# bcsefercik/markerless-robot-camera-calibration

Hardware: AMD Instinct MI355X
Metric: point-cloud frames/sec at 200k pts/frame (higher is better)
Workload: dtype f32

## Files before the change

### include/sv_hip.h

```cpp
#ifndef SV_HIP_H
#define SV_HIP_H

#include <stddef.h>
#include <stdint.h>

#ifdef __cplusplus
extern "C" {
#endif

#define SV_OK 0
#define SV_ERR_INVALID (-1)
#define SV_ERR_WORKSPACE (-2)
#define SV_ERR_HIP (-3)
#define SV_ERR_RANGE (-4)
#define SV_ERR_UNSUPPORTED (-5)

#define SV_ACT_NONE 0
#define SV_ACT_RELU 1
#define SV_ACT_LEAKY_RELU 2

#define SV_POOL_MAX 0
#define SV_POOL_AVG 1

#define SV_REDUCE_MEAN 0
// ... 22 lines not shown
                  sv_stream_t stream);

size_t sv_stride_map_workspace_bytes(int64_t V_in);
int sv_stride_map(const uint64_t* keys_in, int64_t V_in, int level, void* workspace, size_t workspace_bytes,
                  uint64_t* keys_out, int32_t* vcoords_out, int32_t* parent, int32_t* child_start, int32_t* counters,
                  sv_stream_t stream);

int sv_kernel_map_k3(const int32_t* vcoords, int64_t V, int tensor_stride, int dilation, const uint64_t* table_keys,
                     const int32_t* table_vals, int64_t capacity, int32_t* nbr, int64_t ld, uint32_t* mask,
                     sv_stream_t stream);
int sv_kernel_map_down(const uint64_t* keys_fine, const int32_t* parent, int64_t V_fine, int level, int64_t V_coarse,
                       int32_t* nbr, int64_t ld, uint32_t* mask, sv_stream_t stream);
int sv_kernel_map_up(const uint64_t* keys_fine, const int32_t* parent, int64_t V_fine, int level, int32_t* nbr,
                     int64_t ld, uint32_t* mask, sv_stream_t stream);

size_t sv_plan_workspace_bytes(int64_t V);
int sv_plan_build(const int32_t* nbr, int64_t ld, const uint32_t* mask, int K, int64_t V, int64_t nbr_base, void* workspace,
                  size_t workspace_bytes, int32_t* perm, int32_t* nbr_s, uint32_t* submask, int32_t* tile_order,
                  int64_t Vpad, sv_stream_t stream);

#define SV_FRAME_MAX_LEVELS 8
#define SV_FRAME_MAX_CUTS 4
#define SV_FRAME_K3 1
#define SV_FRAME_DOWN 2
#define SV_FRAME_UP 4
#define SV_FRAME_SPLIT 8
#define SV_FRAME_RECORD 16
#define SV_FRAME_REC_HASH 1
#define SV_FRAME_REC_K3 2
#define SV_FRAME_REC_DOWN 3
#define SV_FRAME_REC_UP 4
#define SV_FRAME_REC_SPLIT 5
size_t sv_frame_maps_arena_bytes(int64_t N, int levels);
size_t sv_frame_maps_scratch_bytes(int64_t N);
int sv_frame_maps(const void* coords4, int coords_are_int, int64_t N, int levels, void* arena, size_t arena_bytes, void* scratch,
                  size_t scratch_bytes, int32_t* counters_host, int64_t* layout, sv_stream_t stream);
size_t sv_frame_plans_arena_bytes(const int64_t* V, int levels, int flags, const int32_t* split_cuts);
size_t sv_frame_plans_scratch_bytes(const int64_t* V, int levels);
int sv_frame_plans(const void* const* keys, const void* const* coords, const void* const* parent, const int64_t* V, int levels,
                   int flags, const int32_t* split_cuts, const void* const* k3_nbr, const void* const* k3_mask, void* arena,
                   size_t arena_bytes, void* scratch, size_t scratch_bytes, int64_t* layout, int max_records, sv_stream_t stream);

int sv_conv_fwd(const float* in, int64_t V_in, int64_t in_ld, int Cin, const float* W, int K, int Cout, const int32_t* perm,
                const int32_t* nbr_s, const uint32_t* submask, const int32_t* tile_order, int64_t V_out, int64_t Vpad,
                const float* scale,
                const float* shift, const float* residual, int64_t res_ld, int act, float slope, float* out,
                int64_t out_ld, sv_stream_t stream);
int sv_conv_fwd_acc(const float* in, int64_t V_in, int64_t in_ld, int Cin, const float* W, int K, int Cout, const int32_t* perm,
                    const int32_t* nbr_s, const uint32_t* submask, const int32_t* tile_order, int64_t V_out, int64_t Vpad,
                    const float* acc_init, int64_t acc_ld, const float* scale, const float* shift, const float* residual,
                    int64_t res_ld, int act, float slope, float* out, int64_t out_ld, sv_stream_t stream);
const char* sv_conv_last_instance(void);
int sv_conv_set_dispatch(double want_scale, double tail_fraction);

int sv_pack_weights_bf16(const float* W, int K, int Cin, int Cout, uint16_t* Wp, sv_stream_t stream);
int sv_conv_fwd_bf16(const float* in, int64_t V_in, int64_t in_ld, int Cin, const uint16_t* Wp, int K, int Cout,
                     const int32_t* perm, const int32_t* nbr_s, const uint32_t* submask, const int32_t* tile_order, int64_t V_out,
                     int64_t Vpad, const float* acc_init, int64_t acc_ld, const float* scale, const float* shift,
                     const float* residual, int64_t res_ld, int act, float slope, float* out, int64_t out_ld, sv_stream_t stream);

size_t sv_conv_wgrad_workspace_bytes(int64_t Vpad, int K, int Cin, int Cout);
int sv_conv_wgrad(const float* in, int64_t V_in, int64_t in_ld, int Cin, const float* dy, int64_t V_out, int64_t dy_ld,
                  int Cout, int K, const int32_t* perm, const int32_t* nbr_s, const uint32_t* submask, int64_t Vpad,
                  int accumulate, void* workspace, size_t workspace_bytes, float* dW, sv_stream_t stream);

size_t sv_conv_wgrad_bf16_workspace_bytes(int64_t Vpad, int K, int Cin, int Cout);
int sv_conv_wgrad_bf16(const float* in, int64_t V_in, int64_t in_ld, int Cin, const float* dy, int64_t V_out, int64_t dy_ld,
                       int Cout, int K, const int32_t* perm, const int32_t* nbr_s, const uint32_t* submask, int64_t Vpad,
                       int accumulate, void* workspace, size_t workspace_bytes, float* dW, sv_stream_t stream);

int sv_affine_act(const float* in, int64_t in_ld, int C, int64_t V, const float* scale, const float* shift,
                  const float* residual, int64_t res_ld, int act, float slope, float* out, int64_t out_ld,
                  sv_stream_t stream);

size_t sv_col_stats_workspace_bytes(int64_t N);
int sv_col_stats(const float* x, int64_t ld, int64_t N, int C, const float* sub, void* workspace, size_t workspace_bytes,
                 float* col_min, float* col_max, double* col_sum, float* max_row_norm, sv_stream_t stream);
int sv_center_scale(const float* x, int64_t ld, int64_t N, int C, const float* sub, const float* div, const float* add,
                    float* out, int64_t out_ld, sv_stream_t stream);

int sv_batch_offsets(const uint64_t* keys, int64_t V, int B, int32_t* batch_start, sv_stream_t stream);
int sv_global_pool(const float* F, int64_t ld, int C, const int32_t* batch_start, int B, int mode, float* out,
                   sv_stream_t stream);
int sv_slice_rows(const float* F, int64_t ld, int C, const int64_t* inverse, int64_t N, float* out,
                  sv_stream_t stream);
int sv_slice_argmax(const float* F, int64_t ld, int C, const int64_t* inverse, int64_t N, int64_t* label,
                    float* conf, sv_stream_t stream);
int sv_key_point_predictions(const float* logits, int64_t ld, int C, int64_t N, float conf_th, void* workspace,
                             size_t workspace_bytes, float* prob, int64_t* idx, int32_t* selected, sv_stream_t stream);

int sv_key_point_predictions_batched(const float* logits, int64_t ld, int C, const int64_t* seg_start_host, int G, float conf_th,
                                     void* workspace, size_t workspace_bytes, float* prob, int64_t* idx, int32_t* selected,
                                     sv_stream_t stream);
size_t sv_topk_workspace_bytes(int64_t N, int k);
int sv_topk_indices(const float* x, int64_t ld, int64_t N, int k, void* workspace, size_t workspace_bytes, int64_t* idx,
                    sv_stream_t stream);

int sv_kabsch_batched(const double* ref, const double* tgt, const int32_t* K, int Kmax, int B, double* R, double* t,
                      double* q_wxyz, sv_stream_t stream);
int sv_quat_avg_batched(const double* Q, const double* w, const int32_t* M, int Mmax, int B, double* out,
                        sv_stream_t stream);
int sv_add_metric_batched(const double* points, const int32_t* P, int Pmax, const double* gt_pose,
                          const double* pred_pose, int B, double* add_out, sv_stream_t stream);

size_t sv_icp_workspace_bytes(int64_t S);
int sv_icp_point2point(const float* src, int64_t S, const float* tgt, int64_t T, const double* init_T,
// ... 33 lines not shown
```

### markerless-robot-camera-calibration_amd/_lib.py

```python
import ctypes
import os
from ctypes import c_char_p, c_double, c_float, c_int, c_int64, c_size_t, c_void_p

import torch

_HERE = os.path.dirname(os.path.abspath(__file__))
ABI_VERSION = 4
LIB_PATH = os.environ.get("SVHIP_LIB") or os.path.join(_HERE, "libsvhip.so")

SV_ACT_NONE, SV_ACT_RELU, SV_ACT_LEAKY_RELU = 0, 1, 2
SV_POOL_MAX, SV_POOL_AVG = 0, 1
SV_REDUCE_MEAN, SV_REDUCE_FIRST = 0, 1
SV_TILE_ROWS = 128
SV_ERR_UNSUPPORTED = -5
SV_PN_MAX_LAYERS = 4
SV_PN_MAX_SCALES = 4
SV_BQ_MAX_RADII = 4
SV_COORD_BIAS = 1 << 17
SV_COORD_BITS = 18
SV_MAX_BATCH = 1024
SV_FRAME_MAX_LEVELS, SV_FRAME_MAX_CUTS, SV_FRAME_RECORD = 8, 4, 16
SV_FRAME_K3, SV_FRAME_DOWN, SV_FRAME_UP, SV_FRAME_SPLIT = 1, 2, 4, 8
SV_FRAME_REC_HASH, SV_FRAME_REC_K3, SV_FRAME_REC_DOWN, SV_FRAME_REC_UP, SV_FRAME_REC_SPLIT = 1, 2, 3, 4, 5


class SvHipError(RuntimeError):
    pass


_P = c_void_p
SIGNATURES = {
    "sv_last_error": (c_char_p, []),
    "sv_abi_version": (c_int, []),
    "sv_voxelize_workspace_bytes": (c_size_t, [c_int64]),
    "sv_voxelize": (c_int, [_P, c_int, c_int64, _P, c_size_t, _P, _P, _P, _P, _P, _P, _P]),
    "sv_voxel_reduce": (c_int, [_P, c_int, _P, _P, c_int64, c_int, _P, _P]),
    "sv_hash_build": (c_int, [_P, c_int64, _P, _P, c_int64, _P]),
    "sv_stride_map_workspace_bytes": (c_size_t, [c_int64]),
    "sv_stride_map": (c_int, [_P, c_int64, c_int, _P, c_size_t, _P, _P, _P, _P, _P, _P]),
    "sv_kernel_map_k3": (c_int, [_P, c_int64, c_int, c_int, _P, _P, c_int64, _P, c_int64, _P, _P]),
    "sv_kernel_map_down": (c_int, [_P, _P, c_int64, c_int, c_int64, _P, c_int64, _P, _P]),
    "sv_kernel_map_up": (c_int, [_P, _P, c_int64, c_int, _P, c_int64, _P, _P]),
    "sv_plan_workspace_bytes": (c_size_t, [c_int64]),
    "sv_plan_build": (c_int, [_P, c_int64, _P, c_int, c_int64, c_int64, _P, c_size_t, _P, _P, _P, _P, c_int64, _P]),
    "sv_conv_fwd": (
        c_int,
        [_P, c_int64, c_int64, c_int, _P, c_int, c_int, _P, _P, _P, _P, c_int64, c_int64, _P, _P, _P, c_int64, c_int,
         c_float, _P, c_int64, _P],
    ),
    "sv_conv_fwd_acc": (
        c_int,
        [_P, c_int64, c_int64, c_int, _P, c_int, c_int, _P, _P, _P, _P, c_int64, c_int64, _P, c_int64, _P, _P, _P, c_int64, c_int,
         c_float, _P, c_int64, _P],
    ),
    "sv_pack_weights_bf16": (c_int, [_P, c_int, c_int, c_int, _P, _P]),
    "sv_conv_fwd_bf16": (
        c_int,
        [_P, c_int64, c_int64, c_int, _P, c_int, c_int, _P, _P, _P, _P, c_int64, c_int64, _P, c_int64, _P, _P, _P, c_int64, c_int,
         c_float, _P, c_int64, _P],
    ),
    "sv_conv_wgrad_workspace_bytes": (c_size_t, [c_int64, c_int, c_int, c_int]),
    "sv_conv_wgrad": (
        c_int,
        [_P, c_int64, c_int64, c_int, _P, c_int64, c_int64, c_int, c_int, _P, _P, _P, c_int64, c_int, _P, c_size_t, _P, _P],
    ),
    "sv_conv_wgrad_bf16_workspace_bytes": (c_size_t, [c_int64, c_int, c_int, c_int]),
    "sv_conv_wgrad_bf16": (
        c_int,
        [_P, c_int64, c_int64, c_int, _P, c_int64, c_int64, c_int, c_int, _P, _P, _P, c_int64, c_int, _P, c_size_t, _P, _P],
    ),
    "sv_conv_last_instance": (c_char_p, []),
    "sv_conv_set_dispatch": (c_int, [c_double, c_double]),
    "sv_frame_maps_arena_bytes": (c_size_t, [c_int64, c_int]),
    "sv_frame_maps_scratch_bytes": (c_size_t, [c_int64]),
    "sv_frame_maps": (c_int, [_P, c_int, c_int64, c_int, _P, c_size_t, _P, c_size_t, _P, _P, _P]),
    "sv_frame_plans_arena_bytes": (c_size_t, [_P, c_int, c_int, _P]),
    "sv_frame_plans_scratch_bytes": (c_size_t, [_P, c_int]),
    "sv_frame_plans": (c_int, [_P, _P, _P, _P, c_int, c_int, _P, _P, _P, _P, c_size_t, _P, c_size_t, _P, c_int, _P]),
    "sv_affine_act": (c_int, [_P, c_int64, c_int, c_int64, _P, _P, _P, c_int64, c_int, c_float, _P, c_int64, _P]),
    "sv_col_stats_workspace_bytes": (c_size_t, [c_int64]),
    "sv_col_stats": (c_int, [_P, c_int64, c_int64, c_int, _P, _P, c_size_t, _P, _P, _P, _P, _P]),
    "sv_center_scale": (c_int, [_P, c_int64, c_int64, c_int, _P, _P, _P, _P, c_int64, _P]),
    "sv_batch_offsets": (c_int, [_P, c_int64, c_int, _P, _P]),
    "sv_global_pool": (c_int, [_P, c_int64, c_int, _P, c_int, c_int, _P, _P]),
    "sv_slice_rows": (c_int, [_P, c_int64, c_int, _P, c_int64, _P, _P]),
    "sv_slice_argmax": (c_int, [_P, c_int64, c_int, _P, c_int64, _P, _P, _P]),
    "sv_key_point_predictions": (c_int, [_P, c_int64, c_int, c_int64, c_float, _P, c_size_t, _P, _P, _P, _P]),
    "sv_key_point_predictions_batched": (c_int, [_P, c_int64, c_int, _P, c_int, c_float, _P, c_size_t, _P, _P, _P, _P]),
    "sv_topk_workspace_bytes": (c_size_t, [c_int64, c_int]),
    "sv_topk_indices": (c_int, [_P, c_int64, c_int64, c_int, _P, c_size_t, _P, _P]),
    "sv_kabsch_batched": (c_int, [_P, _P, _P, c_int, c_int, _P, _P, _P, _P]),
    "sv_quat_avg_batched": (c_int, [_P, _P, _P, c_int, c_int, _P, _P]),
    "sv_add_metric_batched": (c_int, [_P, _P, c_int, _P, _P, c_int, _P, _P]),
    "sv_icp_workspace_bytes": (c_size_t, [c_int64]),
    "sv_icp_point2point": (c_int, [_P, c_int64, _P, c_int64, _P, c_double, c_int, c_double, c_double, _P, c_size_t, _P, _P,
                                   _P]),
    "sv_fps": (c_int, [_P, c_int, c_int, c_int, _P, _P, _P]),
    "sv_three_nn_interpolate": (c_int, [_P, _P, _P, c_int, c_int, c_int, c_int, _P, _P]),
    "sv_cluster_workspace_bytes": (c_size_t, [c_int64]),
    "sv_single_linkage_roots": (c_int, [_P, c_int, c_int64, _P, c_int64, c_double, _P, c_size_t, _P, _P, _P]),
    "sv_select_equal": (c_int, [_P, c_int, c_int64, c_int64, _P, _P, _P, _P]),
    "sv_ball_query": (c_int, [_P, _P, c_int, c_int, c_int, c_double, c_int, _P, _P]),
    "sv_fps_segmented": (c_int, [_P, _P, _P, _P, c_int, c_int, _P, _P]),
    "sv_pointnet_sa": (c_int, [_P, _P, _P, _P, c_int, c_int, c_int, c_int, c_int, _P, _P, c_int, _P, _P]),
    "sv_ball_query_multi": (c_int, [_P, _P, c_int, c_int, c_int, c_int, _P, _P, _P, _P]),
    "sv_pointnet_sa_msg": (c_int, [_P, _P, _P, c_int, c_int, c_int, c_int, c_int, _P, _P, _P, _P, _P, _P, _P]),
}

_lib = None


def load():
    global _lib
    if _lib is not None:
        return _lib
    if not os.path.exists(LIB_PATH):
        raise SvHipError(
            f"{LIB_PATH} not found: build it with `python -c 'import __graft_entry__ as g; g.build()'` "
            "(or `make -C markerless-robot-camera-calibration_amd/csrc`). There is no CPU fallback."
        )
    lib = ctypes.CDLL(LIB_PATH)
    lib.sv_abi_version.restype = c_int
    if lib.sv_abi_version() != ABI_VERSION:
        raise SvHipError(f"{LIB_PATH} has C-ABI version {lib.sv_abi_version()}, this package binds version {ABI_VERSION}: "
                         "rebuild it (`python -c 'import __graft_entry__ as g; g.build()'`)")
# ... 53 lines not shown
```

### markerless-robot-camera-calibration_amd/csrc/sv_conv.hip

```cpp
#include <stdarg.h>
#include <stdio.h>
#include <stdlib.h>
#include <type_traits>
#include <algorithm>
#include <vector>

#include "sv_common.h"

namespace sv {

typedef float f32x4 __attribute__((ext_vector_type(4)));

struct ConvParams {
  const float* in;
  int64_t in_ld;
  int Cin;
  const float* W;
  int K;
  int Cout;
  const int32_t* perm;
  const int32_t* nbr_s;
  const uint32_t* submask;
  const int32_t* tile_order;
  int64_t V_out;
// ... 1405 lines not shown
  if (Cout > 128 && (Cout % 192 == 0 || Cout % 96 == 0 || Cout > 2048)) {
    if (Cout % 128 != 0) { list = wide3; n = 3; }
    else if (p.Cin % 128 == 0 && p.vec_a) { list = wide3_128_full; n = 3; }
    else { list = wide3_128; n = 4; }
  }
  else if (Cout > 64) { list = Cout % 64 == 0 ? wide2_64 : wide2; n = 4; }
  else if (Cout > 32) { list = c64; n = 3; }
  else if (Cout > 16) { list = c32; n = 3; }
  else { list = c16; n = 2; }
  static const Candidate f3[] = {{64, 2, 1, 3000, 3}, {32, 2, 1, 0, 3}};
  static const Candidate f32_32[] = {{64, 2, 1, 3000, 32}, {32, 2, 1, 0, 32}};
  static const Candidate f32_64[] = {{32, 4, 1, 1500, 32}, {16, 4, 1, 0, 32}};
  static const Candidate f64_64[] = {{32, 4, 1, 1500, 64}, {16, 4, 1, 0, 64}};
  static const bool no_fused = getenv("SV_CONV_NO_FUSED") != nullptr;
  if (p.K > 1 && !no_fused) {
    if (p.Cin == 3 && Cout > 16 && Cout <= 32) { list = f3; n = 2; }
    else if (p.Cin == 32 && p.vec_a && Cout == 32) { list = f32_32; n = 2; }
    else if (p.Cin == 32 && p.vec_a && Cout == 64) { list = f32_64; n = 2; }
    else if (p.Cin == 64 && p.vec_a && (Cout == 64 || Cout == 128)) { list = f64_64; n = 2; }
  }
  if (const char* f = getenv("SV_CONV_FORCE_RANGE")) {
    long long vmin = 0, vmax = 0;
    int cout = 0;
    Candidate c = {0, 0, 0, 0, 0};
    if (sscanf(f, "%lld:%lld:%d:%d,%d,%d", &vmin, &vmax, &cout, &c.tm, &c.wn, &c.nt) == 6 && p.Vpad >= vmin && p.Vpad <= vmax &&
        p.Cout == cout && p.K > 1)
      return launch_candidate(c, p, stream);
  }
  if (const char* f = getenv("SV_CONV_FORCE_DENSE")) {
    long long vmin = 0;
    int cout = 0;
    Candidate c = {0, 0, 0, 0, 0};
    if (sscanf(f, "%lld:%d:%d,%d,%d", &vmin, &cout, &c.tm, &c.wn, &c.nt) == 5 && p.Vpad >= vmin && p.Cout == cout && p.K == 1)
      return launch_candidate(c, p, stream);
  }
  if (const char* f = getenv("SV_CONV_FORCE")) {
    Candidate c = {0, 0, 0, 0, 0};
    if (sscanf(f, "%d,%d,%d,%d", &c.tm, &c.wn, &c.nt, &c.cpo) >= 3) return launch_candidate(c, p, stream);
  }
  static const double want_scale =
      getenv("SV_CONV_WANT_SCALE") ? atof(getenv("SV_CONV_WANT_SCALE")) : SV_CONV_WANT_SCALE_DEFAULT;
  static const double tail_fraction = getenv("SV_CONV_TAIL") ? atof(getenv("SV_CONV_TAIL")) : SV_CONV_TAIL_DEFAULT;
  const double ws = g_want_scale_override >= 0.0 ? g_want_scale_override : want_scale;
  const double tf = g_tail_override >= 0.0 ? g_tail_override : tail_fraction;
  for (int i = 0; i < n; ++i)
    if ((double)candidate_wgs(list[i], p) >= ws * (double)list[i].want) {
      const Candidate& c = list[i];
      if (c.tm == 64 && c.wn == 4 && c.nt == 3 && c.cpo == 0 && tf > 0.0 &&
          launch_conv_dual<64, 32, 4, 3>(p, stream, tf) == SV_OK)
        return SV_OK;
      return launch_candidate(c, p, stream);
    }
  return launch_candidate(list[n - 1], p, stream);
}

}

using namespace sv;

extern "C" const char* sv_conv_last_instance(void) { return sv::g_last_instance; }

extern "C" int sv_conv_set_dispatch(double want_scale, double tail_fraction) {
  SV_CHECK_ARG(tail_fraction < 1.0, "tail_fraction must be below 1");
  sv::g_want_scale_override = want_scale;
  sv::g_tail_override = tail_fraction;
  return SV_OK;
}

extern "C" int sv_conv_fwd(const float* in, int64_t V_in, int64_t in_ld, int Cin, const float* W, int K, int Cout,
                           const int32_t* perm, const int32_t* nbr_s, const uint32_t* submask,
                           const int32_t* tile_order, int64_t V_out, int64_t Vpad, const float* scale, const float* shift, const float* residual, int64_t res_ld,
                           int act, float slope, float* out, int64_t out_ld, sv_stream_t stream_) {
  return sv_conv_fwd_acc(in, V_in, in_ld, Cin, W, K, Cout, perm, nbr_s, submask, tile_order, V_out, Vpad, nullptr, 0, scale, shift,
                         residual, res_ld, act, slope, out, out_ld, stream_);
}

extern "C" int sv_conv_fwd_acc(const float* in, int64_t V_in, int64_t in_ld, int Cin, const float* W, int K, int Cout,
                               const int32_t* perm, const int32_t* nbr_s, const uint32_t* submask, const int32_t* tile_order,
                               int64_t V_out, int64_t Vpad, const float* acc_init, int64_t acc_ld, const float* scale,
                               const float* shift, const float* residual, int64_t res_ld, int act, float slope, float* out,
                               int64_t out_ld, sv_stream_t stream_) {
  hipStream_t stream = (hipStream_t)stream_;
  SV_CHECK_ARG(!acc_init || acc_ld >= Cout, "acc_init stride too small");
  SV_CHECK_ARG(Cin > 0 && Cout > 0 && K >= 1 && K <= 32, "bad channel / kernel volume");
  SV_CHECK_ARG(V_out >= 0 && Vpad >= V_out && Vpad % PLAN_TILE == 0, "Vpad must be a multiple of 128 >= V_out");
  SV_CHECK_ARG(in_ld >= Cin && out_ld >= Cout, "row strides too small");
  SV_CHECK_ARG(act >= SV_ACT_NONE && act <= SV_ACT_LEAKY_RELU, "bad activation");
  if (V_out == 0) return SV_OK;
  SV_CHECK_ARG(in && W && out, "null pointer");
  SV_CHECK_ARG(V_in >= 1, "V_in = rows of `in` (every index of the plan is below it)");
  const bool has_plan = perm || nbr_s || submask;
  SV_CHECK_ARG(!has_plan || (perm && nbr_s && submask), "perm, nbr_s and submask must be given together");
  SV_CHECK_ARG(has_plan || K == 1, "K > 1 needs a plan");
  SV_CHECK_ARG(!residual || res_ld >= Cout, "residual stride too small");
  ConvParams p;
  p.in = in; p.in_ld = in_ld; p.Cin = Cin; p.W = W; p.K = K; p.Cout = Cout;
  p.perm = perm; p.nbr_s = nbr_s; p.submask = submask; p.tile_order = tile_order; p.V_out = V_out; p.Vpad = Vpad;
  p.scale = scale; p.shift = shift; p.residual = residual; p.res_ld = res_ld;
  p.acc_init = acc_init; p.acc_ld = acc_ld;
  p.act = act; p.slope = slope; p.out = out; p.out_ld = out_ld;
  p.vec_a = (in_ld % 4 == 0) && (Cin % 4 == 0) && (((uintptr_t)in & 15) == 0);
  const uint64_t in_bytes = ((uint64_t)(V_in - 1) * (uint64_t)in_ld + (uint64_t)Cin) * 4u;
  const uint64_t w_bytes = (uint64_t)K * (uint64_t)Cin * (uint64_t)Cout * 4u;
  const uint64_t out_bytes = ((uint64_t)(V_out - 1) * (uint64_t)out_ld + (uint64_t)Cout) * 4u;
  const uint64_t res_bytes = residual ? ((uint64_t)(V_out - 1) * (uint64_t)res_ld + (uint64_t)Cout) * 4u : 0u;
  const uint64_t acc_bytes = acc_init ? ((uint64_t)(V_out - 1) * (uint64_t)acc_ld + (uint64_t)Cout) * 4u : 0u;
  p.buf_ok = in_bytes < BUF_LIMIT && w_bytes < BUF_LIMIT && out_bytes < BUF_LIMIT && res_bytes < BUF_LIMIT &&
             acc_bytes < BUF_LIMIT && (((uintptr_t)perm & 15) == 0);
  p.acc_bytes = p.buf_ok ? (uint32_t)acc_bytes : 0u;
  if (!p.buf_ok && !has_plan && K == 1 && w_bytes < BUF_LIMIT) {
    int64_t ld_max = in_ld > out_ld ? in_ld : out_ld;
    if (residual && res_ld > ld_max) ld_max = res_ld;
    const int64_t rows = (int64_t)((BUF_LIMIT - 4096u) / ((uint64_t)ld_max * 4u)) / PLAN_TILE * PLAN_TILE;
    if (rows >= PLAN_TILE && rows < V_out) {
      for (int64_t r0 = 0; r0 < V_out; r0 += rows) {
        const int64_t n = V_out - r0 < rows ? V_out - r0 : rows;
        const int rc = sv_conv_fwd_acc(in + r0 * in_ld, n, in_ld, Cin, W, K, Cout, nullptr, nullptr, nullptr, nullptr, n,
                                       (n + PLAN_TILE - 1) / PLAN_TILE * PLAN_TILE, acc_init ? acc_init + r0 * acc_ld : nullptr,
                                       acc_ld, scale, shift, residual ? residual + r0 * res_ld : nullptr, res_ld, act, slope,
                                       out + r0 * out_ld, out_ld, stream_);
        if (rc != SV_OK) return rc;
      }
      return SV_OK;
    }
  }
  p.in_bytes = p.buf_ok ? (uint32_t)in_bytes : 0u;
  p.w_bytes = p.buf_ok ? (uint32_t)w_bytes : 0u;
  p.out_bytes = p.buf_ok ? (uint32_t)out_bytes : 0u;
  p.res_bytes = p.buf_ok ? (uint32_t)res_bytes : 0u;
  p.ntiles = 0;
  p.ny = 0;
  p.trace = nullptr;
  p.main_blocks = 0;
  p.main_tiles128 = 0;
  static const bool no_first = getenv("SV_CONV_NO_FIRST") != nullptr;
  static const bool first_valu = getenv("SV_CONV_FIRST_VALU") != nullptr;
  if (has_plan && K > 1 && K <= 27 && Cin == 3 && Cout == 32 && !no_first && !acc_init) {
    if (p.buf_ok && !first_valu) return launch_conv_first_mfma(p, stream);
    return launch_conv_first_layer(p, stream);
  }
  static const bool no_thin = getenv("SV_CONV_NO_THIN") != nullptr;
  if (has_plan && K > 1 && K <= 32 && Cin == 32 && Cout == 32 && p.vec_a && p.buf_ok && !no_thin && !acc_init) return launch_conv_thin(p, stream);
  static const bool no_narrow = getenv("SV_CONV_NO_NARROW") != nullptr;
  if (!has_plan && K == 1 && Cout <= 4 && p.vec_a && Cin >= 64 && !no_narrow && !acc_init) return launch_linear_narrow(p, stream);
  return select_and_launch(p, stream);
}
```

### markerless-robot-camera-calibration_amd/model/robotnet_segmentation.py

```python
import torch.nn as nn

from .. import MinkowskiEngine as ME
from .._lib import SV_ACT_LEAKY_RELU
from ..utils import config
from ._select import pose_backbone, segmentation_backbone

EPS = 1e-6


def _classification_head(UNet, default_classes, class_name):
    class _Head(UNet):
        name = "robotnet"

        def __init__(self, in_channels, out_channels=256, D=3, num_classes=None):
            UNet.__init__(self, in_channels, out_channels, D)
            if num_classes is None:
                num_classes = default_classes()
            self.leaky_relu = ME.MinkowskiLeakyReLU()
            self.regression = nn.Sequential(
                ME.MinkowskiOps.MinkowskiLinear(256, 1024),
                ME.MinkowskiLeakyReLU(),
                ME.MinkowskiOps.MinkowskiLinear(1024, num_classes),
            )
            self.sigm = ME.MinkowskiSigmoid()

        def forward(self, x):
            if isinstance(x, tuple):
                x, _joint_angles = x
            slope = self.leaky_relu.negative_slope
            out = UNet.forward(self, x, final_act=SV_ACT_LEAKY_RELU, final_slope=slope)
            out = self.regression[0].forward_fused(out, act=SV_ACT_LEAKY_RELU,
                                                   slope=self.regression[1].negative_slope)
            return self.regression[2].forward_fused(out)

    _Head.__name__ = _Head.__qualname__ = class_name
    return _Head


def make_robotnet_segmentation(backbone=None):
    return _classification_head(segmentation_backbone(backbone), lambda: config.Config().DATA.classes,
                                "RobotNetSegmentation")


def make_robotnet_vote(backbone=None):
    return _classification_head(pose_backbone(backbone, "ROTATION"),
                                lambda: 2 if config.Config().DATA.data_type == "ee_seg" else 4, "RobotNetVote")


RobotNetSegmentation = make_robotnet_segmentation()
```

### markerless-robot-camera-calibration_amd/nn.py

```python
import math
from ctypes import c_float, c_int, c_int64, c_size_t

import numpy as np
import torch
import torch.nn as nn

from . import _lib, profiling
from ._lib import SV_ACT_LEAKY_RELU, SV_ACT_NONE, SV_ACT_RELU, call, ptr, stream_ptr
from .sparse import SparseTensor, SplitPlan

KERNEL_OFFSET_PERMUTATION = None

import os as _os


def _parse_split_rules(text):
    rules = []
    for part in text.split(";"):
        if part.strip():
            rows, _, cuts = part.partition(":")
            cuts = tuple(int(v) for v in cuts.split(",") if v)
            rules.append((int(rows), cuts[0] if len(cuts) == 1 else cuts))
    return sorted(rules, key=lambda r: -r[0])

# ... 50 lines not shown
        wp = weight_bf16[k0 * Cin * Cout:k1 * Cin * Cout] if weight_bf16 is not None else None
        if i == len(plan.parts) - 1:
            _conv_forward_one(feats, w, sub, V_out, scale, shift, residual, act, slope, out, acc, timed=False, wp=wp)
        else:
            nxt = torch.empty((V_out, Cout), dtype=torch.float32, device=feats.device)
            _conv_forward_one(feats, w, sub, V_out, None, None, None, SV_ACT_NONE, slope, nxt, acc, timed=False, wp=wp)
            acc = nxt
    if t0 is not None:
        timer.stop(t0, _lib.conv_last_instance()[0], K, Cin, Cout, V_out, plan.pairs_device(), level=plan.out_stride,
                   passes=len(plan.parts))
    return out


def _conv_forward_one(feats, weight3, plan, V_out, scale, shift, residual, act, slope, out, acc_init, timed=True, wp=None):
    K, Cin, Cout = weight3.shape
    if plan is None:
        Vpad = (max(V_out, 1) + _lib.SV_TILE_ROWS - 1) // _lib.SV_TILE_ROWS * _lib.SV_TILE_ROWS
    else:
        Vpad = plan.Vpad
    timer = profiling.TIMER if timed else None
    t0 = None
    if timer is not None:
        kname = profiling.conv_kernel_config(Cout, Vpad, Cin, K)
        if timer.want(kname):
            t0 = timer.start()
    res_ld = residual.stride(0) if residual is not None else 0

    log = profiling.INSTANCE_LOG

    acc_ld = acc_init.stride(0) if acc_init is not None else 0

    fn, w_arg = ("sv_conv_fwd_acc", weight3) if wp is None else ("sv_conv_fwd_bf16", wp)

    def launch(f, pl, o, r, v_out, v_pad, a=None):
        call(fn, ptr(f), c_int64(f.shape[0]), c_int64(f.stride(0)), c_int(Cin), ptr(w_arg), c_int(K),
             c_int(Cout), ptr(pl.perm if pl else None), ptr(pl.nbr_s if pl else None), ptr(pl.submask if pl else None),
             ptr(pl.tile_order if pl else None), c_int64(v_out), c_int64(v_pad), ptr(a), c_int64(acc_ld), ptr(scale), ptr(shift),
             ptr(r), c_int64(res_ld), c_int(act), c_float(slope), ptr(o), c_int64(o.stride(0)), stream_ptr())
        if log is not None:
            log.append((*_lib.conv_last_instance(), K, Cin, Cout, v_out))

    parts = plan.chunks(4 * feats.stride(0), 4 * max(out.stride(0), res_ld, acc_ld)) if plan is not None else None
    if parts is None:
        launch(feats, plan, out, residual, V_out, Vpad, acc_init)
    else:
        for sub, i0, i1, o0, o1 in parts:
            launch(feats[i0:i1], sub, out[o0:o1], residual[o0:o1] if residual is not None else None, o1 - o0, sub.Vpad,
                   acc_init[o0:o1] if acc_init is not None else None)
    if t0 is not None:
        timer.stop(t0, _lib.conv_last_instance()[0], K, Cin, Cout, V_out,
                   plan.pairs_device() if plan is not None else None,
                   level=plan.out_stride if plan is not None else None)
    return out


def _wgrad_one(feats, dy, plan, K, Cin, Cout, V_out, dW, accumulate, bf16=False):
    Vpad = (plan.Vpad if plan is not None
            else (max(V_out, 1) + _lib.SV_TILE_ROWS - 1) // _lib.SV_TILE_ROWS * _lib.SV_TILE_ROWS)
    lib = _lib.load()
    fn = "sv_conv_wgrad_bf16" if bf16 else "sv_conv_wgrad"
    nbytes = getattr(lib, fn + "_workspace_bytes")(c_int64(Vpad), c_int(K), c_int(Cin), c_int(Cout))
    ws = torch.empty(max(nbytes, 1), dtype=torch.uint8, device=dy.device)
    rc = getattr(lib, fn)(ptr(feats), c_int64(feats.shape[0]), c_int64(feats.stride(0)), c_int(Cin), ptr(dy),
                          c_int64(V_out), c_int64(dy.stride(0)), c_int(Cout), c_int(K), ptr(plan.perm if plan else None),
                          ptr(plan.nbr_s if plan else None), ptr(plan.submask if plan else None), c_int64(Vpad),
                          c_int(1 if accumulate else 0), ptr(ws), c_size_t(nbytes), ptr(dW), stream_ptr())
    if bf16 and rc == _lib.SV_ERR_UNSUPPORTED:
        return _wgrad_one(feats, dy, plan, K, Cin, Cout, V_out, dW, accumulate)
    _lib._check(rc, fn)
    return fn


def conv_wgrad(feats, dy, plan, K, Cin, Cout, bf16=False, used=None):
    if feats.stride(1) != 1:
        feats = feats.contiguous()
    if dy.stride(1) != 1:
        dy = dy.contiguous()
    V_out = dy.shape[0]
    dW = torch.empty((K, Cin, Cout), dtype=torch.float32, device=dy.device)
    used = set() if used is None else used
    if isinstance(plan, SplitPlan):
        for k0, k1, sub in plan.parts:
            _wgrad_plan(feats, dy, sub, k1 - k0, Cin, Cout, V_out, dW[k0:k1], bf16, used)
    else:
        _wgrad_plan(feats, dy, plan, K, Cin, Cout, V_out, dW, bf16, used)
    return dW


def _wgrad_plan(feats, dy, plan, K, Cin, Cout, V_out, dW, bf16=False, used=None):
    used = set() if used is None else used
    parts = plan.chunks(4 * feats.stride(0), 4 * dy.stride(0)) if plan is not None else None
    if parts is None:
        used.add(_wgrad_one(feats, dy, plan, K, Cin, Cout, V_out, dW, False, bf16))
        return
    for j, (sub, i0, i1, o0, o1) in enumerate(parts):
        used.add(_wgrad_one(feats[i0:i1], dy[o0:o1], sub, K, Cin, Cout, o1 - o0, dW, j > 0, bf16))


def _bf16_fwd_ok(rows, Cin, Cout, K):
    return (Cin % 32 == 0 and Cin >= 64 and Cout % 16 == 0 and Cout >= 64 and K <= 27
            and rows.data_ptr() % 16 == 0 and rows.stride(0) % 4 == 0)


def _train_log(layer, op, fn):
    log = profiling.TRAIN_LOG
    if log is not None:
# ... 517 lines not shown
```

### markerless-robot-camera-calibration_amd/profiling.py

```python
import math

import torch

TIMER = None
INSTANCE_LOG = None
TRAIN_LOG = None

_CANDIDATES = {
    "wide3": [(64, 4, 3, 2500), (32, 4, 3, 1500), (32, 2, 3, 0)],
    "wide3_128": [(64, 4, 3, 2500), (64, 4, 2, 1200), (32, 4, 3, 1200), (16, 4, 3, 0)],
    "wide3_128_full": [(64, 4, 3, 2500), (32, 4, 3, 1200), (16, 4, 3, 0)],
    "wide2": [(128, 4, 2, 1300), (64, 4, 2, 1500), (32, 4, 2, 1500), (32, 2, 2, 0)],
    "wide2_64": [(128, 4, 2, 1300), (64, 4, 2, 1500), (32, 4, 2, 1500), (16, 4, 1, 0)],
    "c64": [(64, 4, 1, 1500), (32, 4, 1, 1500), (16, 4, 1, 0)],
    "c32": [(128, 2, 1, 1500), (64, 2, 1, 1500), (32, 2, 1, 0)],
    "c16": [(128, 1, 1, 600), (64, 1, 1, 0)],
}


import os

CONV_TAIL_FRACTION = float(os.environ.get("SV_CONV_TAIL", "0.15"))
CONV_WANT_SCALE = float(os.environ.get("SV_CONV_WANT_SCALE", "0.3"))

# ... 20 lines not shown
        else:
            fused = _FUSED.get((Cin, Cout))
    if fused is not None:
        cands = fused
    elif Cout > 128 and (Cout % 192 == 0 or Cout % 96 == 0 or Cout > 2048):
        if Cout % 128 != 0:
            cands = _CANDIDATES["wide3"]
        else:
            cands = _CANDIDATES["wide3_128_full" if (Cin is not None and Cin % 128 == 0) else "wide3_128"]
    elif Cout > 64:
        cands = _CANDIDATES["wide2_64" if Cout % 64 == 0 else "wide2"]
    elif Cout > 32:
        cands = _CANDIDATES["c64"]
    elif Cout > 16:
        cands = _CANDIDATES["c32"]
    else:
        cands = _CANDIDATES["c16"]
    suffix = f", fused {Cin}>" if fused is not None else ">"
    for tm, wn, nt, want in cands:
        tn = wn * nt * 16
        if (Vpad // tm) * ((Cout + tn - 1) // tn) >= want * CONV_WANT_SCALE:
            if ((tm, wn, nt) == (64, 4, 3) and fused is None and K > 1 and Cin is not None and Cin % 4 == 0
                    and Cout % tn == 0 and CONV_TAIL_FRACTION > 0 and int((Vpad // 128) * CONV_TAIL_FRACTION) >= 1):
                return "conv_fwd_dual_kernel<64, 32, 4, 3>"
            return f"conv_fwd_kernel<{tm}, {wn}, {nt}{suffix}"
    tm, wn, nt, _ = cands[-1]
    return f"conv_fwd_kernel<{tm}, {wn}, {nt}{suffix}"


class KernelTimer:
    def __init__(self, capacity=0):
        self.records = []
        self.enabled = True
        self.only = None
        self._pool = [torch.cuda.Event(enable_timing=True) for _ in range(capacity)]
        self._next = 0
        self._first_of_frame = False

    def _event(self):
        if self._next < len(self._pool):
            e = self._pool[self._next]
            self._next += 1
            return e
        return torch.cuda.Event(enable_timing=True)

    def want(self, kernel):
        return self.enabled and (self.only is None or kernel in self.only)

    def start(self):
        e = self._event()
        e.record()
        return e

    def stop(self, start_evt, kernel, K, Cin, Cout, V_out, pairs_dev, level=None, passes=1):
        e = self._event()
        e.record()
        self.records.append((kernel, K, Cin, Cout, V_out, pairs_dev, start_evt, e, self._first_of_frame, level, passes))
        self._first_of_frame = False

    def frame_boundary(self):
        self._first_of_frame = True

    def clear(self):
        self.records = []

    @staticmethod
    def layer_key(kernel, K, Cin, Cout, V_out, level=None):
        where = f"s{level}" if level is not None else f"~2^{int(round(math.log2(max(V_out, 1))))}"
        return (kernel, K, Cin, Cout, where)

    def summarize(self, by_layer=False):
        out = {}
        for kernel, K, Cin, Cout, V_out, pairs_dev, s, e, first, level, passes in self.records:
            if first:
                continue
            P = int(pairs_dev.item()) if pairs_dev is not None else V_out
            ms = s.elapsed_time(e)
            key = self.layer_key(kernel, K, Cin, Cout, V_out, level) if by_layer else kernel
            d = out.setdefault(key, {"launches": 0, "ms": 0.0, "flops": 0.0, "bytes": 0.0, "rows": 0.0, "kernel_launches": 0})
            d["rows"] += V_out
            d["launches"] += 1
            d["kernel_launches"] += passes
            d["ms"] += ms
            d["flops"] += 2.0 * P * Cin * Cout
            d["bytes"] += P * (4.0 * Cin + 8) + 4.0 * V_out * Cout + 4.0 * K * Cin * Cout
        return out


def pass_gflop(fn):
    global TIMER
    saved, TIMER = TIMER, KernelTimer()
    try:
        fn()
        torch.cuda.synchronize()
        return sum(d["flops"] for d in TIMER.summarize().values()) / 1e9
    finally:
        TIMER = saved
```

Before: 73.84.

## Fuse final 1x1 conv and two-layer MLP head into one HIP kernel

Adds sv_head_fwd, a single kernel that runs the final pointwise conv (Cin0->256), the 256->1024 linear and the 1024->C linear with leaky-ReLU, using MFMA f32 and keeping intermediates in LDS. The segmentation head uses it when the shapes match and the row count is large enough. This removes the global-memory round trips of the 256- and 1024-wide activations and two extra launches. The cost is a complex kernel whose LDS footprint limits occupancy, and which recomputes in chunks with a scalar final reduction.

Result: no change. 73.82, median of 3 (-0.0%).

```diff
diff --git a/include/sv_hip.h b/include/sv_hip.h
--- a/include/sv_hip.h
+++ b/include/sv_hip.h
@@ -98,6 +98,9 @@
                     int64_t res_ld, int act, float slope, float* out, int64_t out_ld, sv_stream_t stream);
 const char* sv_conv_last_instance(void);
 int sv_conv_set_dispatch(double want_scale, double tail_fraction);
+int sv_head_fwd(const float* in, int64_t V, int64_t in_ld, int Cin0, const float* W0, const float* b0, float slope0, int C1,
+                const float* W1, const float* b1, float slope1, int C2, const float* W2, const float* b2, int C, float* out,
+                int64_t out_ld, sv_stream_t stream);
 
 int sv_pack_weights_bf16(const float* W, int K, int Cin, int Cout, uint16_t* Wp, sv_stream_t stream);
 int sv_conv_fwd_bf16(const float* in, int64_t V_in, int64_t in_ld, int Cin, const uint16_t* Wp, int K, int Cout,
diff --git a/markerless-robot-camera-calibration_amd/_lib.py b/markerless-robot-camera-calibration_amd/_lib.py
--- a/markerless-robot-camera-calibration_amd/_lib.py
+++ b/markerless-robot-camera-calibration_amd/_lib.py
@@ -71,6 +71,8 @@
     ),
     "sv_conv_last_instance": (c_char_p, []),
     "sv_conv_set_dispatch": (c_int, [c_double, c_double]),
+    "sv_head_fwd": (c_int, [_P, c_int64, c_int64, c_int, _P, _P, c_float, c_int, _P, _P, c_float, c_int, _P, _P, c_int, _P,
+                            c_int64, _P]),
     "sv_frame_maps_arena_bytes": (c_size_t, [c_int64, c_int]),
     "sv_frame_maps_scratch_bytes": (c_size_t, [c_int64]),
     "sv_frame_maps": (c_int, [_P, c_int, c_int64, c_int, _P, c_size_t, _P, c_size_t, _P, _P, _P]),
diff --git a/markerless-robot-camera-calibration_amd/csrc/sv_conv.hip b/markerless-robot-camera-calibration_amd/csrc/sv_conv.hip
--- a/markerless-robot-camera-calibration_amd/csrc/sv_conv.hip
+++ b/markerless-robot-camera-calibration_amd/csrc/sv_conv.hip
@@ -1481,6 +1481,223 @@
       return launch_candidate(c, p, stream);
     }
   return launch_candidate(list[n - 1], p, stream);
+}
+
+struct HeadParams {
+  const float* in;
+  int64_t in_ld;
+  int Cin0;
+  int64_t V;
+  const float* W0;
+  const float* b0;
+  float slope0;
+  const float* W1;
+  const float* b1;
+  float slope1;
+  const float* W2;
+  const float* b2;
+  float* out;
+  int64_t out_ld;
+  uint32_t in_bytes, w0_bytes;
+};
+constexpr int HEAD_TM = 64, HEAD_C1 = 256, HEAD_C2 = 1024;
+constexpr int HEAD_KC = 64;
+constexpr int HEAD_SX = 66;
+constexpr int HEAD_NC = 64;
+static_assert(2 * HEAD_TM * HEAD_SX <= HEAD_TM * HEAD_C1, "the staged X fits the H1 region");
+__device__ __forceinline__ int head_h1_idx(int r, int c) { return r * HEAD_C1 + (c ^ ((r & 15) << 1)); }
+
+template <int C, bool FULL>
+__global__ __launch_bounds__(256, 2) void sv_head_kernel(HeadParams p) {
+  __shared__ __attribute__((aligned(16))) float h1[HEAD_TM * HEAD_C1];
+  __shared__ __attribute__((aligned(16))) float h2[HEAD_NC * HEAD_TM];
+  const int tid = threadIdx.x;
+  const int lane = tid & 63;
+  const int wid = __builtin_amdgcn_readfirstlane(tid >> 6);
+  const int li = lane & 15, lq = lane >> 4;
+  const int64_t row0 = (int64_t)blockIdx.x * HEAD_TM;
+  const int Cin0 = p.Cin0;
+  const __amdgpu_buffer_rsrc_t rsrc_in = __builtin_amdgcn_make_buffer_rsrc((void*)p.in, 0, (int)p.in_bytes, 0x00020000);
+  const __amdgpu_buffer_rsrc_t rsrc_w0 = __builtin_amdgcn_make_buffer_rsrc((void*)p.W0, 0, (int)p.w0_bytes, 0x00020000);
+  const __amdgpu_buffer_rsrc_t rsrc_w1 =
+      __builtin_amdgcn_make_buffer_rsrc((void*)p.W1, 0, HEAD_C1 * HEAD_C2 * 4, 0x00020000);
+
+  const int col0 = 64 * wid + 4 * li;
+  const int xc = (tid & 15) * 4, xr = tid >> 4;
+  uint32_t xoff[4];
+#pragma unroll
+  for (int j = 0; j < 4; ++j) {
+    const int64_t r = row0 + xr + 16 * j;
+    xoff[j] = r < p.V ? (uint32_t)r * (uint32_t)(p.in_ld * 4) + (uint32_t)xc * 4u : BUF_ABSENT;
+  }
+  f32x4 xg[4];
+  auto load_x = [&](int c0) {
+#pragma unroll
+    for (int j = 0; j < 4; ++j) xg[j] = buffer_load_floats<4>(rsrc_in, xoff[j], (uint32_t)c0 * 4u);
+  };
+  auto store_x = [&](float* xs) {
+#pragma unroll
+    for (int j = 0; j < 4; ++j) {
+      float2* d = (float2*)(xs + (xr + 16 * j) * HEAD_SX + xc);
+      d[0] = make_float2(xg[j][0], xg[j][1]);
+      d[1] = make_float2(xg[j][2], xg[j][3]);
+    }
+  };
+  const uint32_t b0_lane = (uint32_t)(lq * HEAD_C1 + col0) * 4u;
+  f32x4 b0v[HEAD_KC / 4];
+  auto load_b0 = [&](int c0) {
+#pragma unroll
+    for (int ks = 0; ks < HEAD_KC / 4; ++ks)
+      b0v[ks] = buffer_load_floats<4>(rsrc_w0, b0_lane, (uint32_t)(c0 + 4 * ks) * (uint32_t)(HEAD_C1 * 4));
+  };
+  f32x4 acc0[4][4];
+#pragma unroll
+  for (int s = 0; s < 4; ++s)
+#pragma unroll
+    for (int n = 0; n < 4; ++n) acc0[s][n] = (f32x4){0.f, 0.f, 0.f, 0.f};
+  float bias0[4];
+#pragma unroll
+  for (int n = 0; n < 4; ++n) bias0[n] = p.b0[col0 + n];
+
+  const int nsteps = (Cin0 + HEAD_KC - 1) / HEAD_KC;
+  load_x(0);
+  load_b0(0);
+  store_x(h1);
+  __syncthreads();
+  int buf = 0;
+  for (int st = 0; st < nsteps; ++st) {
+    const int c0 = st * HEAD_KC;
+    const bool more = st + 1 < nsteps;
+    if (more) load_x(c0 + HEAD_KC);
+    const float* a_base = h1 + buf * (HEAD_TM * HEAD_SX) + li * HEAD_SX + lq;
+    const int ksteps = (min(HEAD_KC, Cin0 - c0) + 3) >> 2;
+    float a_cur[4];
+#pragma unroll
+    for (int s = 0; s < 4; ++s) a_cur[s] = a_base[s * 16 * HEAD_SX];
+#pragma unroll
+    for (int ks = 0; ks < HEAD_KC / 4; ++ks) {
+      if (FULL || ks < ksteps) {
+        float a_nx[4];
+        if (ks + 1 < HEAD_KC / 4) {
+#pragma unroll
+          for (int s = 0; s < 4; ++s) a_nx[s] = a_base[s * 16 * HEAD_SX + (ks + 1) * 4];
+        }
+#pragma unroll
+        for (int s = 0; s < 4; ++s)
+#pragma unroll
+          for (int n = 0; n < 4; ++n) acc0[s][n] = __builtin_amdgcn_mfma_f32_16x16x4f32(a_cur[s], b0v[ks][n], acc0[s][n], 0, 0, 0);
+        if (ks + 1 < HEAD_KC / 4) {
+#pragma unroll
+          for (int s = 0; s < 4; ++s) a_cur[s] = a_nx[s];
+        }
+      }
+      if (more) b0v[ks] = buffer_load_floats<4>(rsrc_w0, b0_lane, (uint32_t)(c0 + HEAD_KC + 4 * ks) * (uint32_t)(HEAD_C1 * 4));
+    }
+    if (more) store_x(h1 + (buf ^ 1) * (HEAD_TM * HEAD_SX));
+    __syncthreads();
+    buf ^= 1;
+  }
+
+  const int wm = wid >> 1, wn = wid & 1;
+  const uint32_t b1_lane = (uint32_t)(lq * HEAD_C2 + 32 * wn + 2 * li) * 4u;
+  typedef float f32x2 __attribute__((ext_vector_type(2)));
+  f32x2 b1v[HEAD_C1 / 4];
+#pragma unroll
+  for (int ks = 0; ks < HEAD_C1 / 4; ++ks)
+    b1v[ks] = buffer_load_floats<2>(rsrc_w1, b1_lane, (uint32_t)(4 * ks * HEAD_C2) * 4u);
+
+  const float slope0 = p.slope0;
+#pragma unroll
+  for (int s = 0; s < 4; ++s)
+#pragma unroll
+    for (int reg = 0; reg < 4; ++reg) {
+      float v[4];
+#pragma unroll
+      for (int n = 0; n < 4; ++n) {
+        float t = __builtin_fmaf(acc0[s][n][reg], 1.0f, bias0[n]) + -0.0f;
+        v[n] = t > 0.f ? t : t * slope0;
+      }
+      const int r = 16 * s + 4 * lq + reg;
+      *(float2*)(h1 + head_h1_idx(r, col0)) = make_float2(v[0], v[1]);
+      *(float2*)(h1 + head_h1_idx(r, col0 + 2)) = make_float2(v[2], v[3]);
+    }
+  __syncthreads();
+
+  const float* a_row[8];
+#pragma unroll
+  for (int k8 = 0; k8 < 8; ++k8) a_row[k8] = h1 + (32 * wm + li) * HEAD_C1 + ((4 * k8 + lq) ^ (li << 1));
+  const float slope1 = p.slope1;
+  const int jw = wid < C ? wid : 0;
+  float y = 0.0f;
+  constexpr int NCH = HEAD_C2 / HEAD_NC;
+  constexpr int PF = 2;
+  for (int ch = 0; ch < NCH; ++ch) {
+    const int cb = ch * HEAD_NC;
+    const bool more = ch + 1 < NCH;
+    float bias1[2];
+#pragma unroll
+    for (int n = 0; n < 2; ++n) bias1[n] = p.b1[cb + 32 * wn + 2 * li + n];
+    f32x4 acc1[2][2];
+#pragma unroll
+    for (int s = 0; s < 2; ++s)
+#pragma unroll
+      for (int n = 0; n < 2; ++n) acc1[s][n] = (f32x4){0.f, 0.f, 0.f, 0.f};
+    float a_ring[PF + 1][2];
+#pragma unroll
+    for (int d = 0; d < PF; ++d)
+#pragma unroll
+      for (int s = 0; s < 2; ++s) a_ring[d][s] = a_row[d & 7][32 * (d >> 3) + 4096 * s];
+#pragma unroll
+    for (int ks = 0; ks < HEAD_C1 / 4; ++ks) {
+      if (ks + PF < HEAD_C1 / 4) {
+        const int kn = ks + PF;
+#pragma unroll
+        for (int s = 0; s < 2; ++s) a_ring[kn % (PF + 1)][s] = a_row[kn & 7][32 * (kn >> 3) + 4096 * s];
+      }
+#pragma unroll
+      for (int s = 0; s < 2; ++s)
+#pragma unroll
+        for (int n = 0; n < 2; ++n)
+          acc1[s][n] = __builtin_amdgcn_mfma_f32_16x16x4f32(a_ring[ks % (PF + 1)][s], b1v[ks][n], acc1[s][n], 0, 0, 0);
+      if (more) b1v[ks] = buffer_load_floats<2>(rsrc_w1, b1_lane, (uint32_t)(4 * ks * HEAD_C2 + cb + HEAD_NC) * 4u);
+    }
+    __syncthreads();
+#pragma unroll
+    for (int s = 0; s < 2; ++s)
+#pragma unroll
+      for (int n = 0; n < 2; ++n) {
+        float4 v;
+        float* vp = (float*)&v;
+#pragma unroll
+        for (int reg = 0; reg < 4; ++reg) {
+          float t = __builtin_fmaf(acc1[s][n][reg], 1.0f, bias1[n]) + -0.0f;
+          vp[reg] = t > 0.f ? t : t * slope1;
+        }
+        *(float4*)(h2 + (32 * wn + 2 * li + n) * HEAD_TM + 32 * wm + 16 * s + 4 * lq) = v;
+      }
+    __syncthreads();
+    if (wid < C) {
+      const float* w2 = p.W2 + (int64_t)cb * C + jw;
+#pragma unroll 16
+      for (int c = 0; c < HEAD_NC; ++c) y = __builtin_fmaf(h2[c * HEAD_TM + lane], w2[c * C], y);
+    }
+  }
+  const int64_t r = row0 + lane;
+  if (wid < C && r < p.V) p.out[r * p.out_ld + jw] = y + p.b2[jw];
+}
+
+template <int C>
+static int launch_head_c(const HeadParams& p, hipStream_t stream) {
+  const unsigned grid = (unsigned)((p.V + HEAD_TM - 1) / HEAD_TM);
+  if (p.Cin0 % HEAD_KC == 0) {
+    hipLaunchKernelGGL((sv_head_kernel<C, true>), dim3(grid), dim3(256), 0, stream, p);
+    note_instance("sv_head_kernel<%d>|fast=1,ring=0,full=1", C);
+  } else {
+    hipLaunchKernelGGL((sv_head_kernel<C, false>), dim3(grid), dim3(256), 0, stream, p);
+    note_instance("sv_head_kernel<%d>|fast=1,ring=0,full=0", C);
+  }
+  SV_LAUNCH_CHECK();
+  return SV_OK;
 }
 
 }
@@ -1574,3 +1791,41 @@
   if (!has_plan && K == 1 && Cout <= 4 && p.vec_a && Cin >= 64 && !no_narrow && !acc_init) return launch_linear_narrow(p, stream);
   return select_and_launch(p, stream);
 }
+
+extern "C" int sv_head_fwd(const float* in, int64_t V, int64_t in_ld, int Cin0, const float* W0, const float* b0, float slope0,
+                           int C1, const float* W1, const float* b1, float slope1, int C2, const float* W2, const float* b2,
+                           int C, float* out, int64_t out_ld, sv_stream_t stream_) {
+  hipStream_t stream = (hipStream_t)stream_;
+  SV_CHECK_ARG(V >= 0 && Cin0 > 0 && C1 > 0 && C2 > 0 && C > 0, "bad shape");
+  SV_CHECK_ARG(in_ld >= Cin0 && out_ld >= C, "row strides too small");
+  if (Cin0 % 4 != 0 || C1 != HEAD_C1 || C2 != HEAD_C2 || C > 4 || in_ld % 4 != 0 || ((uintptr_t)in & 15) != 0 ||
+      (uint64_t)Cin0 * HEAD_C1 * 4u >= BUF_LIMIT) {
+    sv::set_error("sv_head_fwd: Cin0 = %d, C1 = %d, C2 = %d, C = %d, in_ld = %lld outside the fused head (Cin0 %% 4 == 0, "
+                  "C1 = 256, C2 = 1024, C <= 4, 16-byte aligned rows)", Cin0, C1, C2, C, (long long)in_ld);
+    return SV_ERR_UNSUPPORTED;
+  }
+  if (V == 0) return SV_OK;
+  SV_CHECK_ARG(in && W0 && b0 && W1 && b1 && W2 && b2 && out, "null pointer");
+  const int64_t rows_max = (int64_t)((BUF_LIMIT - 4096u) / ((uint64_t)in_ld * 4u)) / HEAD_TM * HEAD_TM;
+  SV_CHECK_ARG(rows_max >= HEAD_TM, "row stride too large");
+  for (int64_t r0 = 0; r0 < V; r0 += rows_max) {
+    const int64_t n = V - r0 < rows_max ? V - r0 : rows_max;
+    HeadParams p;
+    p.in = in + r0 * in_ld; p.in_ld = in_ld; p.Cin0 = Cin0; p.V = n;
+    p.W0 = W0; p.b0 = b0; p.slope0 = slope0;
+    p.W1 = W1; p.b1 = b1; p.slope1 = slope1;
+    p.W2 = W2; p.b2 = b2;
+    p.out = out + r0 * out_ld; p.out_ld = out_ld;
+    p.in_bytes = (uint32_t)(((uint64_t)(n - 1) * (uint64_t)in_ld + (uint64_t)Cin0) * 4u);
+    p.w0_bytes = (uint32_t)((uint64_t)Cin0 * HEAD_C1 * 4u);
+    int rc;
+    switch (C) {
+      case 1: rc = launch_head_c<1>(p, stream); break;
+      case 2: rc = launch_head_c<2>(p, stream); break;
+      case 3: rc = launch_head_c<3>(p, stream); break;
+      default: rc = launch_head_c<4>(p, stream); break;
+    }
+    if (rc != SV_OK) return rc;
+  }
+  return SV_OK;
+}
diff --git a/markerless-robot-camera-calibration_amd/model/robotnet_segmentation.py b/markerless-robot-camera-calibration_amd/model/robotnet_segmentation.py
--- a/markerless-robot-camera-calibration_amd/model/robotnet_segmentation.py
+++ b/markerless-robot-camera-calibration_amd/model/robotnet_segmentation.py
@@ -1,9 +1,11 @@
 import torch.nn as nn
 
 from .. import MinkowskiEngine as ME
+from .. import nn as svnn
 from .._lib import SV_ACT_LEAKY_RELU
 from ..utils import config
 from ._select import pose_backbone, segmentation_backbone
+from .backbone.minkunet import MinkUNetBase
 
 EPS = 1e-6
 
@@ -28,9 +30,17 @@
             if isinstance(x, tuple):
                 x, _joint_angles = x
             slope = self.leaky_relu.negative_slope
-            out = UNet.forward(self, x, final_act=SV_ACT_LEAKY_RELU, final_slope=slope)
-            out = self.regression[0].forward_fused(out, act=SV_ACT_LEAKY_RELU,
-                                                   slope=self.regression[1].negative_slope)
+            slope1 = self.regression[1].negative_slope
+            if UNet.forward is MinkUNetBase.forward and svnn.head_fusable(self.final, self.regression[0],
+                                                                          self.regression[2], x.F.shape[0]):
+                feats = self.forward_except_final(x)
+                out = svnn.head_forward(feats, self.final, slope, self.regression[0], slope1, self.regression[2])
+                if out is not None:
+                    return out
+                out = self.final.forward_fused(feats, act=SV_ACT_LEAKY_RELU, slope=slope)
+            else:
+                out = UNet.forward(self, x, final_act=SV_ACT_LEAKY_RELU, final_slope=slope)
+            out = self.regression[0].forward_fused(out, act=SV_ACT_LEAKY_RELU, slope=slope1)
             return self.regression[2].forward_fused(out)
 
     _Head.__name__ = _Head.__qualname__ = class_name
diff --git a/markerless-robot-camera-calibration_amd/nn.py b/markerless-robot-camera-calibration_amd/nn.py
--- a/markerless-robot-camera-calibration_amd/nn.py
+++ b/markerless-robot-camera-calibration_amd/nn.py
@@ -126,6 +126,52 @@
                    plan.pairs_device() if plan is not None else None,
                    level=plan.out_stride if plan is not None else None)
     return out
+
+
+HEAD_FUSE_MIN_ROWS = int(_os.environ.get("MRCC_HEAD_FUSE_MIN_ROWS", str(1 << 17)))
+
+
+def head_fusable(final, lin0, lin2, rows):
+    mods = (final, lin0, lin2)
+    if rows < HEAD_FUSE_MIN_ROWS or any(m.training or m.compute_precision != "fp32" for m in mods):
+        return False
+    if final.kernel_volume != 1 or final.stride != 1 or final.transposed or final.bias is None:
+        return False
+    if lin0.linear.bias is None or lin2.linear.bias is None:
+        return False
+    return (final.out_channels == lin0.linear.in_features == 256 and lin0.linear.out_features == lin2.linear.in_features
+            == 1024 and lin2.linear.out_features <= 4)
+
+
+def head_forward(x, final, slope0, lin0, slope1, lin2, out=None):
+    feats = x.F if isinstance(x, SparseTensor) else x
+    if feats.stride(1) != 1:
+        feats = feats.contiguous()
+    V, Cin0 = feats.shape
+    w0 = final.weight3().detach()
+    w1, w2 = lin0.weight3(), lin2.weight3()
+    C = w2.shape[2]
+    if out is None:
+        out = torch.empty((V, C), dtype=torch.float32, device=feats.device)
+    name = f"sv_head_kernel<{C}>"
+    timer = profiling.TIMER
+    t0 = timer.start() if timer is not None and timer.want(name) else None
+    rc = _lib.load().sv_head_fwd(ptr(feats), c_int64(V), c_int64(feats.stride(0)), c_int(Cin0), ptr(w0),
+                                 ptr(final.bias.detach()), c_float(slope0), c_int(w1.shape[1]), ptr(w1),
+                                 ptr(lin0.linear.bias.detach()), c_float(slope1), c_int(w1.shape[2]), ptr(w2),
+                                 ptr(lin2.linear.bias.detach()), c_int(C), ptr(out), c_int64(out.stride(0)), stream_ptr())
+    if rc == _lib.SV_ERR_UNSUPPORTED:
+        return None
+    _lib._check(rc, "sv_head_fwd")
+    log = profiling.INSTANCE_LOG
+    if log is not None:
+        log.append((*_lib.conv_last_instance(), 1, Cin0, C, V))
+    if t0 is not None:
+        C1, C2 = w1.shape[1], w1.shape[2]
+        flops = 2.0 * V * (Cin0 * C1 + C1 * C2 + C2 * C)
+        nbytes = sum(V * (4.0 * a + 8) + 4.0 * V * b + 4.0 * a * b for a, b in ((Cin0, C1), (C1, C2), (C2, C)))
+        timer.stop(t0, name, 1, Cin0, C, V, None, flops=flops, nbytes=nbytes)
+    return x.new(out) if isinstance(x, SparseTensor) else out
 
 
 def _wgrad_one(feats, dy, plan, K, Cin, Cout, V_out, dW, accumulate, bf16=False):
diff --git a/markerless-robot-camera-calibration_amd/profiling.py b/markerless-robot-camera-calibration_amd/profiling.py
--- a/markerless-robot-camera-calibration_amd/profiling.py
+++ b/markerless-robot-camera-calibration_amd/profiling.py
@@ -96,10 +96,11 @@
         e.record()
         return e
 
-    def stop(self, start_evt, kernel, K, Cin, Cout, V_out, pairs_dev, level=None, passes=1):
+    def stop(self, start_evt, kernel, K, Cin, Cout, V_out, pairs_dev, level=None, passes=1, flops=None, nbytes=None):
         e = self._event()
         e.record()
-        self.records.append((kernel, K, Cin, Cout, V_out, pairs_dev, start_evt, e, self._first_of_frame, level, passes))
+        self.records.append((kernel, K, Cin, Cout, V_out, pairs_dev, start_evt, e, self._first_of_frame, level, passes,
+                             flops, nbytes))
         self._first_of_frame = False
 
     def frame_boundary(self):
@@ -115,7 +116,7 @@
 
     def summarize(self, by_layer=False):
         out = {}
-        for kernel, K, Cin, Cout, V_out, pairs_dev, s, e, first, level, passes in self.records:
+        for kernel, K, Cin, Cout, V_out, pairs_dev, s, e, first, level, passes, flops, nbytes in self.records:
             if first:
                 continue
             P = int(pairs_dev.item()) if pairs_dev is not None else V_out
@@ -126,8 +127,8 @@
             d["launches"] += 1
             d["kernel_launches"] += passes
             d["ms"] += ms
-            d["flops"] += 2.0 * P * Cin * Cout
-            d["bytes"] += P * (4.0 * Cin + 8) + 4.0 * V_out * Cout + 4.0 * K * Cin * Cout
+            d["flops"] += 2.0 * P * Cin * Cout if flops is None else flops
+            d["bytes"] += P * (4.0 * Cin + 8) + 4.0 * V_out * Cout + 4.0 * K * Cin * Cout if nbytes is None else nbytes
         return out
 
 
```
